# ZooMEISTER/vickers-hardness-Unet

Measured on AMD Instinct MI355X. Metric: 512x512 images/sec (train fwd+bwd), higher is better.
Workload: dtype bf16

## Files before the change

include/vk_unet.h:

```cpp
#ifndef VK_UNET_H
#define VK_UNET_H

#include <stddef.h>
#include <stdint.h>

#ifdef __cplusplus
extern "C" {
#endif

#define VK_ABI_VERSION 1
#define VK_STATS_REPLICAS 32

typedef enum { VK_F32 = 0, VK_BF16 = 1, VK_F16 = 2 } vk_dtype;

enum { VK_OK = 0, VK_ERR_ARG = -1, VK_ERR_STATE = -2, VK_ERR_UNSUPPORTED = -3 };

int vk_version(void);
const char* vk_last_error_string(void);
int vk_has_gfx950_code(void);
int vk_probe_mfma_rate(int iters, int waves_per_simd, float* sink, double* flops_out, void* stream);
int vk_set_reserved_cus(int n);
int vk_debug_hold_cus(int workgroups, int threads, int lds_bytes, int microseconds, const void* traffic, size_t traffic_bytes,
                      float* sink, void* stream);

int vk_debug_set_stamp_buffer(void* device_buffer);
int vk_prof_enable(int on);
int vk_prof_collect(char* buf, size_t buflen);


typedef struct {
  const void* ptr;
  int C;
  int up;
  const float* scale;
  const float* shift;
  int relu;
} vk_src;

typedef struct {
  vk_dtype dtype;
  int N, H, W;
  int Ho, Wo;
  int K;
  int R, S, stride, pad;
  int transposed;
  vk_src src0, src1;
} vk_conv_desc;

int vk_conv_fwd(const vk_conv_desc* d, const void* w, void* y, void* y1, int split_k1, int accumulate,
                double* stats, void* stream);

int vk_conv_dgrad_pool2(const vk_conv_desc* d, const void* w, void* y_half, void* y1, int split_k1, int accumulate,
                        void* stream);

int vk_halo_pack(vk_dtype dtype, int rows, int red, const void* src, void* dst, void* stream);
int vk_conv_uses_halo_pack(const vk_conv_desc* d);
int vk_conv_fwd_packed(const vk_conv_desc* d, const void* w_halo, void* y, void* y1, int split_k1, int accumulate, double* stats,
                       void* stream);

#define VK_SPLITK_WORKSPACE_BYTES (32u << 20)
int vk_conv_fwd_splitk(const vk_conv_desc* d, const void* w_halo, void* y, void* workspace, size_t workspace_bytes, void* stream);

typedef struct {
  const void* z;
  const float* scale;
  const float* shift;
  double* sums;
  const void* mask;
  int accumulate;
} vk_bnr;

int vk_conv_dgrad_fused(const vk_conv_desc* d, const void* w, void* y, void* y1, int split_k1, int pool2, const vk_bnr* bnr,
                        void* stream);

int vk_conv1x1_fwd(const vk_conv_desc* d, const void* w, void* y, int accumulate, double* stats, void* stream);
int vk_conv1x1_wgrad(const vk_conv_desc* d, const void* dz, float* dw, void* workspace, size_t workspace_bytes, void* stream);

int vk_stem_fwd(vk_dtype dtype, int N, int H, int W, const void* x4, const void* wp, void* y, double* stats,
                void* stream);

#define VK_WGRAD_WORKSPACE_BYTES (64u << 20)
int vk_conv_wgrad(const vk_conv_desc* d, const void* dz, float* dw, void* workspace, size_t workspace_bytes, void* stream);
#define VK_WGRAD_BATCH_TABLE_BYTES (128u << 10)
int vk_conv_wgrad_batch_supports(const vk_conv_desc* d);
int vk_conv_wgrad_batch(const vk_conv_desc* descs, const void* const* dz, float* const* dw, int n, int workgroups, void* tables,
                        size_t tables_bytes, void* workspace, size_t workspace_bytes, void* stream);
int vk_stem_wgrad(vk_dtype dtype, int N, int H, int W, const void* x4, const void* dz, float* dw_krsc3, void* workspace,
                  size_t workspace_bytes, void* stream);
int vk_stem_wgrad_bn(vk_dtype dtype, int N, int H, int W, const void* x4, const void* g, const void* z, const float* coef_abc,
                     float* dw_krsc3, void* workspace, size_t workspace_bytes, void* stream);
int vk_stem_dgrad(vk_dtype dtype, int N, int H, int W, const void* g, const void* z, const float* coef_abc, const float* w_krsc3,
                  float* dx, void* stream);

typedef struct {
  int h, w;
  int src_stride;
  int size;
  int nh, nw;
  int top, left;
  int pad_value;
} vk_letterbox_desc;

int vk_letterbox_preprocess(const vk_letterbox_desc* d, const uint8_t* bgr, float* x_nchw, void* stream);
int vk_letterbox_postprocess_mask(const vk_letterbox_desc* d, const float* logits, float thresh, uint8_t* mask_hw, void* stream);
int vk_letterbox_postprocess_prob(const vk_letterbox_desc* d, const float* logits, float* prob_hw, void* stream);
int vk_letterbox_postprocess_labels(const vk_letterbox_desc* d, int C, const float* logits, uint8_t* labels_hw, void* stream);
int vk_letterbox_postprocess_mask_multi(const vk_letterbox_desc* d, int C, const float* logits, float thresh, uint8_t* masks_chw,
                                        void* stream);
int vk_letterbox_postprocess_prob_multi(const vk_letterbox_desc* d, int C, int mode, const float* logits, float* probs_chw, void* stream);

typedef struct {
  int h, w;
  float bin_thresh;
  int morph_kernel;
  int open_iter;
  int close_iter;
  int min_area;
  int max_components;
} vk_geom_desc;

typedef struct {
  int label;
  int area;
  int box[8];
  float cx, cy;
  float rw, rh;
  float ux, uy;
  int hull_n;
  int reserved;
  double d1, d2, d_mean;
} vk_geom_det;

int64_t vk_geom_workspace_bytes(const vk_geom_desc* d, int batch);
int vk_geom_minarearect(const vk_geom_desc* d, int batch, const float* prob, uint8_t* clean, vk_geom_det* dets, int* counts,
                        void* workspace, size_t workspace_bytes, void* stream);

typedef struct {
  int label;
  int area;
  int box[8];
  float cx, cy;
  int valid;
  int branch;
  int n_candidates;
  int contour_n;
  int hull_n;
  int flags;
  double quality;
  double d1, d2, d_mean;
} vk_geom_quad;

int vk_geom_quadrilateral(const vk_geom_desc* d, int fit_outset_px, int batch, const float* prob, uint8_t* clean, vk_geom_quad* dets,
                          int* counts, void* workspace, size_t workspace_bytes, void* stream);

typedef struct {
  int d4;
  int rotate;
  float cos_a, sin_a;
  int photo;
  float alpha, beta;
  int blur_ksize;
  float noise_scale;
  uint32_t noise_seed;
  int clahe_limit;
} vk_aug_params;

#define VK_AUG_TABLE_INTS (256 + 4097 + 4097)
size_t vk_augment_workspace_bytes(int n, int size);

int vk_letterbox_u8(const vk_letterbox_desc* d, const uint8_t* bgr, uint8_t* rgb_sq, void* stream);
int vk_letterbox_mask_u8(const vk_letterbox_desc* d, const uint8_t* mask_hw, uint8_t* mask_sq, void* stream);
int vk_augment_batch(int n, int size, int n_items, const uint8_t* images_rgb, const uint8_t* masks, const int* index_dev,
                     const vk_aug_params* params_host, void* params_dev, const int* color_tables, void* workspace,
// ... 198 lines not shown
```

vickers-hardness-unet_amd/_lib.py:

```python
from __future__ import annotations

import ctypes as C
import os
import subprocess
from pathlib import Path

PKG_DIR = Path(__file__).resolve().parent
LIB_PATH = Path(os.environ["VK_LIB"]) if os.environ.get("VK_LIB") else PKG_DIR / "libvkunet.so"
CSRC = PKG_DIR / "csrc"

VK_F32, VK_BF16, VK_F16 = 0, 1, 2
VK_LOSS_BINARY, VK_LOSS_MULTILABEL, VK_LOSS_MULTICLASS = 0, 1, 2
VK_ENC_RESNET18, VK_ENC_RESNET34, VK_ENC_RESNET50 = 18, 34, 50


class VkError(RuntimeError):
    pass


class vk_src(C.Structure):
    _fields_ = [("ptr", C.c_void_p), ("C", C.c_int), ("up", C.c_int), ("scale", C.c_void_p),
                ("shift", C.c_void_p), ("relu", C.c_int)]


# ... 12 lines not shown
    _fields_ = [("h", C.c_int), ("w", C.c_int), ("src_stride", C.c_int), ("size", C.c_int), ("nh", C.c_int),
                ("nw", C.c_int), ("top", C.c_int), ("left", C.c_int), ("pad_value", C.c_int)]


class vk_geom_desc(C.Structure):
    _fields_ = [("h", C.c_int), ("w", C.c_int), ("bin_thresh", C.c_float), ("morph_kernel", C.c_int), ("open_iter", C.c_int),
                ("close_iter", C.c_int), ("min_area", C.c_int), ("max_components", C.c_int)]


class vk_geom_det(C.Structure):
    _fields_ = [("label", C.c_int), ("area", C.c_int), ("box", C.c_int * 8), ("cx", C.c_float), ("cy", C.c_float),
                ("rw", C.c_float), ("rh", C.c_float), ("ux", C.c_float), ("uy", C.c_float), ("hull_n", C.c_int),
                ("reserved", C.c_int), ("d1", C.c_double), ("d2", C.c_double), ("d_mean", C.c_double)]


class vk_geom_quad(C.Structure):
    _fields_ = [("label", C.c_int), ("area", C.c_int), ("box", C.c_int * 8), ("cx", C.c_float), ("cy", C.c_float),
                ("valid", C.c_int), ("branch", C.c_int), ("n_candidates", C.c_int), ("contour_n", C.c_int), ("hull_n", C.c_int),
                ("flags", C.c_int), ("quality", C.c_double), ("d1", C.c_double), ("d2", C.c_double), ("d_mean", C.c_double)]


class vk_aug_params(C.Structure):
    _fields_ = [("d4", C.c_int), ("rotate", C.c_int), ("cos_a", C.c_float), ("sin_a", C.c_float), ("photo", C.c_int),
                ("alpha", C.c_float), ("beta", C.c_float), ("blur_ksize", C.c_int), ("noise_scale", C.c_float),
                ("noise_seed", C.c_uint32), ("clahe_limit", C.c_int)]


class vk_seg_loss_cfg(C.Structure):
    _fields_ = [("struct_size", C.c_uint32), ("mode", C.c_int32), ("terms", C.c_uint32), ("has_ignore", C.c_int32),
                ("ignore_index", C.c_int32), ("w_pix", C.c_float), ("w_focal", C.c_float), ("w_dice", C.c_float),
                ("w_jaccard", C.c_float), ("w_tversky", C.c_float), ("pix_smooth", C.c_float), ("pix_denom_valid", C.c_int32),
                ("has_pos_weight", C.c_int32), ("pos_weight", C.c_float * 16), ("focal_has_alpha", C.c_int32),
                ("focal_alpha", C.c_float), ("focal_gamma", C.c_float),
                ("dice_smooth", C.c_float), ("dice_eps", C.c_float), ("dice_log", C.c_int32), ("dice_classes", C.c_uint32),
                ("jaccard_smooth", C.c_float), ("jaccard_eps", C.c_float), ("jaccard_log", C.c_int32), ("jaccard_classes", C.c_uint32),
                ("tversky_smooth", C.c_float), ("tversky_eps", C.c_float), ("tversky_log", C.c_int32), ("tversky_classes", C.c_uint32),
                ("tversky_alpha", C.c_float), ("tversky_beta", C.c_float), ("tversky_gamma", C.c_float),
                ("w_mcc", C.c_float), ("mcc_eps", C.c_float)]


class vk_lovasz_cfg(C.Structure):
    _fields_ = [("struct_size", C.c_uint32), ("mode", C.c_int32), ("per_image", C.c_int32), ("has_ignore", C.c_int32),
                ("ignore_index", C.c_int32)]


class vk_unet_config(C.Structure):
    _fields_ = [("N", C.c_int), ("size", C.c_int), ("dtype", C.c_int), ("training", C.c_int), ("width", C.c_int)]


class vk_tensor_info(C.Structure):
    _fields_ = [("name", C.c_char * 96), ("kind", C.c_int), ("dims", C.c_int * 4), ("ndim", C.c_int),
                ("offset", C.c_int64), ("numel", C.c_int64)]


vp, ci, cf, cd, sz, i64 = C.c_void_p, C.c_int, C.c_float, C.c_double, C.c_size_t, C.c_int64
P = C.POINTER

SIGNATURES = {
    "vk_version": (ci, []),
    "vk_last_error_string": (C.c_char_p, []),
    "vk_has_gfx950_code": (ci, []),
    "vk_probe_mfma_rate": (ci, [ci, ci, vp, P(C.c_double), vp]),
    "vk_set_reserved_cus": (ci, [ci]),
    "vk_debug_hold_cus": (ci, [ci, ci, ci, ci, vp, sz, vp, vp]),
    "vk_debug_set_stamp_buffer": (ci, [vp]),
    "vk_prof_enable": (ci, [ci]),
    "vk_prof_collect": (ci, [C.c_char_p, sz]),
    "vk_conv_fwd": (ci, [P(vk_conv_desc), vp, vp, vp, ci, ci, vp, vp]),
    "vk_conv_dgrad_pool2": (ci, [P(vk_conv_desc), vp, vp, vp, ci, ci, vp]),
    "vk_conv_dgrad_fused": (ci, [P(vk_conv_desc), vp, vp, vp, ci, ci, P(vk_bnr), vp]),
    "vk_head_bwd_fused": (ci, [ci, ci, ci, ci, P(vk_src), vp, vp, vp, vp, vp, P(vk_bnr), vp, sz, vp]),
    "vk_halo_pack": (ci, [ci, ci, ci, vp, vp, vp]),
    "vk_conv_uses_halo_pack": (ci, [P(vk_conv_desc)]),
    "vk_conv_fwd_packed": (ci, [P(vk_conv_desc), vp, vp, vp, ci, ci, vp, vp]),
    "vk_conv_fwd_splitk": (ci, [P(vk_conv_desc), vp, vp, vp, sz, vp]),
    "vk_stem_fwd": (ci, [ci, ci, ci, ci, vp, vp, vp, vp, vp]),
    "vk_conv_wgrad": (ci, [P(vk_conv_desc), vp, vp, vp, sz, vp]),
    "vk_conv1x1_fwd": (ci, [P(vk_conv_desc), vp, vp, ci, vp, vp]),
    "vk_conv1x1_wgrad": (ci, [P(vk_conv_desc), vp, vp, vp, sz, vp]),
    "vk_conv_wgrad_batch_supports": (ci, [P(vk_conv_desc)]),
    "vk_conv_wgrad_batch": (ci, [P(vk_conv_desc), P(vp), P(vp), ci, ci, vp, sz, vp, sz, vp]),
    "vk_stem_wgrad": (ci, [ci, ci, ci, ci, vp, vp, vp, vp, sz, vp]),
    "vk_stem_wgrad_bn": (ci, [ci, ci, ci, ci, vp, vp, vp, vp, vp, vp, sz, vp]),
    "vk_stem_dgrad": (ci, [ci, ci, ci, ci, vp, vp, vp, vp, vp, vp]),
    "vk_letterbox_preprocess": (ci, [P(vk_letterbox_desc), vp, vp, vp]),
    "vk_letterbox_postprocess_mask": (ci, [P(vk_letterbox_desc), vp, cf, vp, vp]),
    "vk_letterbox_postprocess_prob": (ci, [P(vk_letterbox_desc), vp, vp, vp]),
    "vk_letterbox_postprocess_labels": (ci, [P(vk_letterbox_desc), ci, vp, vp, vp]),
    "vk_letterbox_postprocess_mask_multi": (ci, [P(vk_letterbox_desc), ci, vp, cf, vp, vp]),
    "vk_letterbox_postprocess_prob_multi": (ci, [P(vk_letterbox_desc), ci, ci, vp, vp, vp]),
    "vk_geom_workspace_bytes": (i64, [P(vk_geom_desc), ci]),
    "vk_geom_minarearect": (ci, [P(vk_geom_desc), ci, vp, vp, vp, vp, vp, sz, vp]),
    "vk_geom_quadrilateral": (ci, [P(vk_geom_desc), ci, ci, vp, vp, vp, vp, vp, sz, vp]),
    "vk_letterbox_u8": (ci, [P(vk_letterbox_desc), vp, vp, vp]),
    "vk_letterbox_mask_u8": (ci, [P(vk_letterbox_desc), vp, vp, vp]),
    "vk_augment_workspace_bytes": (C.c_size_t, [ci, ci]),
    "vk_augment_batch": (ci, [ci, ci, ci, vp, vp, vp, P(vk_aug_params), vp, vp, vp, C.c_size_t, vp, vp, vp]),
    "vk_input_transform": (ci, [ci, ci, ci, ci, vp, vp, vp]),
    "vk_bn_finalize": (ci, [ci, ci, vp, cd, vp, vp, vp, vp, cf, cf, vp, vp, vp, vp, vp]),
    "vk_bn_relu_maxpool": (ci, [ci, ci, ci, ci, ci, vp, vp, vp, vp, vp, vp]),
    "vk_maxpool_bwd": (ci, [ci, ci, ci, ci, ci, vp, vp, vp, vp]),
    "vk_maxpool_bwd_bn_reduce": (ci, [ci, ci, ci, ci, ci, vp, vp, vp, vp, vp, vp, vp, vp]),
    "vk_bn_add_relu": (ci, [ci, sz, ci, vp, vp, vp, vp, vp, vp, vp, vp]),
    "vk_bn_bwd_reduce": (ci, [ci, sz, ci, vp, vp, ci, vp, vp, vp, vp, vp]),
    "vk_bn_bwd_coeffs": (ci, [ci, vp, cd, vp, vp, vp, vp, vp, vp, vp]),
    "vk_bn_bwd_coeffs_frozen": (ci, [ci, vp, vp, vp, vp, vp, vp, vp, vp]),
    "vk_bn_bwd_apply": (ci, [ci, sz, ci, vp, vp, ci, vp, vp, vp, vp, vp, vp, ci, vp]),
    "vk_bn_bwd_apply_fused": (ci, [ci, sz, ci, vp, vp, ci, vp, vp, vp, vp, cd, vp, vp, vp, vp, vp, vp, vp, ci, vp]),
    "vk_upsample2x_bwd": (ci, [ci, ci, ci, ci, ci, vp, vp, ci, vp]),
    "vk_head_fwd": (ci, [ci, ci, ci, ci, P(vk_src), vp, vp, vp, vp]),
    "vk_dec4_tail_eval": (ci, [ci, ci, ci, ci, P(vk_src), vp, vp, vp, vp, vp, vp, vp, vp, vp, vp]),
    "vk_head_bwd": (ci, [ci, ci, ci, ci, P(vk_src), vp, vp, vp, vp, vp, vp, sz, vp]),
    "vk_bce_dice_loss": (ci, [sz, vp, vp, vp, vp, vp, cf, cf, cf, vp]),
    "vk_head_fwd_multi": (ci, [ci, ci, ci, ci, ci, P(vk_src), vp, vp, vp, vp]),
    "vk_head_multi_workspace_bytes": (sz, [ci]),
    "vk_head_bwd_multi": (ci, [ci, ci, ci, ci, ci, P(vk_src), vp, vp, vp, vp, vp, P(vk_bnr), vp, sz, vp]),
    "vk_multi_loss_workspace_bytes": (sz, [ci, ci, ci]),
    "vk_multilabel_loss": (ci, [ci, ci, ci, vp, vp, vp, sz, vp, vp, cf, cf, cf, vp]),
    "vk_multiclass_loss": (ci, [ci, ci, ci, vp, vp, vp, sz, vp, vp, cf, cf, cf, vp]),
    "vk_seg_loss_cfg_size": (sz, []),
    "vk_seg_loss_workspace_bytes": (sz, [ci, ci, ci]),
    "vk_seg_loss": (ci, [P(vk_seg_loss_cfg), ci, ci, ci, vp, vp, vp, sz, vp, vp, cf, vp]),
    "vk_lovasz_cfg_size": (sz, []),
    "vk_lovasz_workspace_bytes": (sz, [P(vk_lovasz_cfg), ci, ci, ci]),
    "vk_lovasz_loss": (ci, [P(vk_lovasz_cfg), ci, ci, ci, vp, vp, vp, sz, vp, vp, cf, ci, vp]),
    "vk_lovasz_flat_workspace_bytes": (sz, [ci, i64]),
    "vk_lovasz_flat": (ci, [vp, vp, ci, i64, vp, sz, vp, vp, vp, vp]),
    "vk_seg_metrics_workspace_bytes": (C.c_size_t, [ci]),
    "vk_seg_metrics": (ci, [ci, sz, vp, vp, ci, cf, cf, vp, sz, vp, vp]),
    "vk_seg_metrics_multi_workspace_bytes": (sz, [ci, ci]),
    "vk_seg_metrics_multi": (ci, [ci, ci, ci, sz, vp, vp, ci, cf, cf, vp, sz, vp, vp, vp, vp]),
    "vk_adamw_step": (ci, [sz, vp, vp, vp, vp, cf, cf, cf, cf, cf, ci, cf, vp, vp, ci, vp]),
    "vk_amp_check_inf": (ci, [sz, vp, vp, vp]),
    "vk_amp_unscale_check": (ci, [sz, vp, vp, vp, vp]),
    "vk_adamw_step_amp": (ci, [sz, vp, vp, vp, vp, cf, cf, cf, cf, cf, vp, cf, vp, vp, vp, vp, ci, vp]),
    "vk_adamw_segment_blocks": (ci, [ci, P(i64), P(C.c_int32), ci]),
    "vk_adamw_step_amp_segments": (ci, [ci, vp, ci, vp, vp, vp, vp, vp, cf, cf, cf, cf, cf, vp, cf, vp, vp, vp, vp]),
    "vk_unet_create": (ci, [P(vk_unet_config), P(vp)]),
    "vk_unet_create_ex": (ci, [P(vk_unet_config), ci, P(vp)]),
    "vk_unet_num_classes": (ci, [vp]),
    "vk_unet_create_enc": (ci, [P(vk_unet_config), ci, ci, P(vp)]),
    "vk_unet_encoder": (ci, [vp]),
    "vk_unet_destroy": (None, [vp]),
    "vk_unet_set_side_stream": (ci, [vp, ci]),
    "vk_unet_num_tensors": (ci, [vp]),
    "vk_unet_tensor_info": (ci, [vp, ci, P(vk_tensor_info)]),
    "vk_unet_param_numel": (i64, [vp]),
    "vk_unet_buffer_numel": (i64, [vp]),
    "vk_unet_workspace_bytes": (i64, [vp]),
    "vk_unet_num_buckets": (ci, [vp]),
    "vk_unet_bucket_range": (ci, [vp, ci, P(i64), P(i64)]),
    "vk_unet_bind": (ci, [vp, vp, vp, vp, vp, vp, sz]),
    "vk_unet_refresh_weights": (ci, [vp, vp]),
    "vk_unet_forward": (ci, [vp, vp, vp, ci, vp]),
    "vk_unet_loss": (ci, [vp, vp, vp, vp, cf, cf, cf, vp]),
    "vk_unet_loss_ex": (ci, [vp, ci, vp, vp, vp, cf, cf, cf, vp]),
    "vk_unet_loss_cfg": (ci, [vp, P(vk_seg_loss_cfg), vp, vp, vp, cf, vp]),
    "vk_unet_loss_lovasz": (ci, [vp, P(vk_seg_loss_cfg), P(vk_lovasz_cfg), cf, vp, vp, vp, sz, vp, cf, vp]),
    "vk_unet_backward": (ci, [vp, vp, ci, ci, vp]),
    "vk_unet_set_trainable": (ci, [vp, P(C.c_uint8), ci]),
    "vk_unet_set_bn_frozen": (ci, [vp, P(C.c_uint8), ci]),
    "vk_unet_set_input_grad": (ci, [vp, vp]),
    "vk_unet_zero_grad": (ci, [vp, vp]),
    "vk_unet_debug_tensor": (ci, [vp, C.c_char_p, P(vp), P(ci * 4)]),
    "vk_comm_unique_id": (ci, [vp]),
    "vk_comm_init": (ci, [ci, ci, vp, P(vp)]),
# ... 78 lines not shown
```

vickers-hardness-unet_amd/csrc/engine.hip:

```cpp
#include <stdarg.h>
#include <stdio.h>
#include <stdlib.h>
#include <string.h>

#include <algorithm>
#include <atomic>
#include <map>
#include <mutex>
#include <string>
#include <vector>

#include "vk_common.h"

namespace vkh {
static thread_local char g_err[512] = "";
void set_error(const char* fmt, ...) {
  va_list ap;
  va_start(ap, fmt);
  vsnprintf(g_err, sizeof(g_err), fmt, ap);
  va_end(ap);
}

struct ProfRec {
  std::string tag;
// ... 1234 lines not shown
                  void* g_out, int g_acc, hipStream_t st) {
  static const int maxc = getenv("VK_BN_APPLY_FUSED_MAXC") ? atoi(getenv("VK_BN_APPLY_FUSED_MAXC")) : VK_BN_APPLY_FUSED_MAXC_DEFAULT;
  if (frozen(h, b)) {
    if (trains(h, b.g_t) || trains(h, b.b_t))
      RET_IF(vk_bn_bwd_coeffs_frozen(C, b.bsums, h->params + b.g_off, b.mean, b.invstd, dgamma_of(h, b), dbeta_of(h, b), b.coef, st));
    return vk_bn_bwd_apply(h->cfg.dtype, pixels, C, dy, z, mask_mode, b.scale, b.shift, mask_src, b.coef, dz, g_out, g_acc, st);
  }
  if (C <= maxc)
    return vk_bn_bwd_apply_fused(h->cfg.dtype, pixels, C, dy, z, mask_mode, b.scale, b.shift, mask_src, b.bsums, b.count, h->params + b.g_off,
                                 b.mean, b.invstd, dgamma_of(h, b), dbeta_of(h, b), dz, g_out, g_acc, st);
  RET_IF(vk_bn_bwd_coeffs(C, b.bsums, b.count, h->params + b.g_off, b.mean, b.invstd, dgamma_of(h, b), dbeta_of(h, b), b.coef, st));
  return vk_bn_bwd_apply(h->cfg.dtype, pixels, C, dy, z, mask_mode, b.scale, b.shift, mask_src, b.coef, dz, g_out, g_acc, st);
}

int bn_relu_bwd_inplace(vk_unet* h, ConvL& c, bool prereduced, hipStream_t st) {
  BnL& b = h->bns[c.bn];
  const size_t pixels = (size_t)h->cfg.N * c.Hout * c.Wout;
  if (!prereduced && bn_sums_needed(h, b)) RET_IF(vk_bn_bwd_reduce(h->cfg.dtype, pixels, c.K, c.g, c.z, 1, b.scale, b.shift, nullptr, b.bsums, st));
  return bn_bwd_phase2(h, b, c.K, pixels, c.g, c.z, prereduced ? 0 : 1, nullptr, c.g, nullptr, 0, st);
}

int wgrad_stream(vk_unet* h, hipStream_t st, hipStream_t* out) {
  *out = st;
  if (!h->side) return VK_OK;
  VK_CHECK_HIP(hipEventRecord(h->ev_fork, st));
  VK_CHECK_HIP(hipStreamWaitEvent(h->side, h->ev_fork, 0));
  h->side_dirty = true;
  *out = h->side;
  return VK_OK;
}

int join_side(vk_unet* h, hipStream_t st) {
  if (!h->side || !h->side_dirty) return VK_OK;
  VK_CHECK_HIP(hipEventRecord(h->ev_join, h->side));
  VK_CHECK_HIP(hipStreamWaitEvent(st, h->ev_join, 0));
  h->side_dirty = false;
  return VK_OK;
}

int conv_wgrad(vk_unet* h, ConvL& c, const vk_src& s0, const vk_src& s1, hipStream_t st) {
  vk_conv_desc d = conv_desc(h, c, s0, s1);
  if (!h->side && vk::wgrad_batch_supports(&d)) {
    h->pending.push_back(vk_unet::WItem{d, c.g, h->grads + c.w_off});
    return VK_OK;
  }
  hipStream_t ws;
  RET_IF(wgrad_stream(h, st, &ws));
  return vk_conv_wgrad(&d, c.g, h->grads + c.w_off, h->ws + h->off_wslab, VK_WGRAD_WORKSPACE_BYTES, ws);
}

vk_bnr bnr_of(vk_unet* h, ConvL& target) {
  BnL& b = h->bns[target.bn];
  vk_bnr r;
  r.z = target.z; r.scale = b.scale; r.shift = b.shift; r.sums = b.bsums; r.mask = nullptr; r.accumulate = 0;
  return r;
}

vk_conv_desc dgrad_desc(vk_unet* h, ConvL& c) {
  vk_conv_desc d;
  d.dtype = h->cfg.dtype;
  d.N = h->cfg.N; d.H = c.Hout; d.W = c.Wout; d.Ho = c.Hin; d.Wo = c.Win;
  d.K = c.Cin; d.R = c.R; d.S = c.R; d.stride = c.stride; d.pad = c.pad; d.transposed = 1;
  vk_src s;
  s.ptr = c.g; s.C = c.K; s.up = 0; s.scale = nullptr; s.shift = nullptr; s.relu = 0;
  d.src0 = s;
  d.src1 = null_src();
  return d;
}

int conv_dgrad_into(vk_unet* h, ConvL& c, ConvL& into, bool* fused, hipStream_t st) {
  vk_conv_desc d = dgrad_desc(h, c);
  if (on_1x1(c)) {
    *fused = false;
    return vk_conv1x1_fwd(&d, dgrad_weights(h, c), into.g, 0, nullptr, st);
  }
  vk_bnr r = bnr_of(h, into);
  int rc = getenv("VK_NO_BNR_FUSION") ? VK_ERR_UNSUPPORTED : vk_conv_dgrad_fused(&d, dgrad_weights(h, c), into.g, nullptr, 0, 0, &r, st);
  *fused = rc == VK_OK;
  if (rc != VK_ERR_UNSUPPORTED) return rc;
  if (c.halo_dg) return vk_conv_fwd_packed(&d, dgrad_weights(h, c), into.g, nullptr, 0, 0, nullptr, st);
  return vk_conv_fwd(&d, dgrad_weights(h, c), into.g, nullptr, 0, 0, nullptr, st);
}

int conv_dgrad(vk_unet* h, ConvL& c, void* y, void* y1, int split, int accumulate, hipStream_t st) {
  vk_conv_desc d;
  d.dtype = h->cfg.dtype;
  d.N = h->cfg.N; d.H = c.Hout; d.W = c.Wout; d.Ho = c.Hin; d.Wo = c.Win;
  d.K = c.Cin; d.R = c.R; d.S = c.R; d.stride = c.stride; d.pad = c.pad; d.transposed = 1;
  vk_src s;
  s.ptr = c.g; s.C = c.K; s.up = 0; s.scale = nullptr; s.shift = nullptr; s.relu = 0;
  d.src0 = s;
  d.src1 = null_src();
  if (on_1x1(c) && !split) return vk_conv1x1_fwd(&d, dgrad_weights(h, c), y, accumulate, nullptr, st);
  if (c.halo_dg) return vk_conv_fwd_packed(&d, dgrad_weights(h, c), y, y1, split, accumulate, nullptr, st);
  return vk_conv_fwd(&d, dgrad_weights(h, c), y, y1, split, accumulate, nullptr, st);
}

int backward_decoder(vk_unet* h, int i, hipStream_t st) {
  DecL& d = h->decs[i];
  ConvL& c1 = h->convs[d.conv1];
  ConvL& c2 = h->convs[d.conv2];
  const int N = h->cfg.N;
  ConvL& stem = h->convs[h->stem_conv];
  Act xprev, skip{nullptr, 0, nullptr, nullptr, 0};
  void* g_prev;
  if (i == 0) {
    BlockL& f5 = h->blocks[h->layer_last_block[3]];
    xprev = Act{f5.out, f5.C, nullptr, nullptr, 0};
    g_prev = f5.gout;
  } else {
    ConvL& pc2 = h->convs[h->decs[i - 1].conv2];
    xprev = bn_act(h, pc2);
    g_prev = pc2.g;
  }
  void* g_skip = nullptr;
  if (i <= 2) {
    BlockL& fb = h->blocks[h->layer_last_block[2 - i]];
    skip = Act{fb.out, fb.C, nullptr, nullptr, 0};
    g_skip = fb.gout;
  } else if (i == 3) {
    skip = bn_act(h, stem);
    g_skip = stem.g;
  }
  const BnL& bn1 = h->bns[c1.bn];
  if (!need_from(h, h->bns[c2.bn].rank)) {
    if (i > 0) h->g_prereduced[h->decs[i - 1].conv2] = 0;
    return VK_OK;
  }
  RET_IF(bn_relu_bwd_inplace(h, c2, h->g_prereduced[d.conv2] != 0, st));
  const bool into1 = need_from(h, bn1.rank);
  bool fused1 = false;
  if (into1) RET_IF(conv_dgrad_into(h, c2, c1, &fused1, st));
  if (trains(h, c2.w_t)) RET_IF(conv_wgrad(h, c2, to_src(bn_act(h, c1)), null_src(), st));
  if (i > 0) h->g_prereduced[h->decs[i - 1].conv2] = 0;
  if (!into1) return VK_OK;
  RET_IF(bn_relu_bwd_inplace(h, c1, fused1, st));
  if (need_from(h, c1.rank + 1)) {
    vk_conv_desc dd = dgrad_desc(h, c1);
    vk_bnr r;
    const bool want_bnr = i > 0 && !getenv("VK_NO_BNR_FUSION");
    if (want_bnr) r = bnr_of(h, h->convs[h->decs[i - 1].conv2]);
    const int rc = vk_conv_dgrad_fused(&dd, dgrad_weights(h, c1), g_prev, d.Cskip ? g_skip : nullptr, d.Cskip ? d.Cup : 0, 1,
                                       want_bnr ? &r : nullptr, st);
    if (rc == VK_OK && want_bnr) h->g_prereduced[h->decs[i - 1].conv2] = 1;
    if (rc != VK_OK && rc != VK_ERR_UNSUPPORTED) return rc;
    if (rc == VK_ERR_UNSUPPORTED) {
      void* dup = h->ws + h->off_dup;
      if (d.Cskip) RET_IF(conv_dgrad(h, c1, dup, g_skip, d.Cup, 0, st));
      else RET_IF(conv_dgrad(h, c1, dup, nullptr, 0, 0, st));
      RET_IF(vk_upsample2x_bwd(h->cfg.dtype, N, d.H, d.W, d.Cup, dup, g_prev, 0, st));
    }
  }
  if (!trains(h, c1.w_t)) return VK_OK;
  return conv_wgrad(h, c1, to_src(xprev, 1), d.Cskip ? to_src(skip) : null_src(), st);
}

int backward_block(vk_unet* h, int bi, hipStream_t st) {
  BlockL& k = h->blocks[bi];
  ConvL& c1 = h->convs[k.conv1];
  ConvL& c2 = h->convs[k.conv2];
  BnL& b2 = h->bns[c2.bn];
  const vk_dtype dt = h->cfg.dtype;
  const size_t pixels = (size_t)h->cfg.N * k.Hout * k.Wout;
  if (!need_from(h, b2.rank)) {
    h->tail_prereduced[(size_t)bi] = 0;
    return VK_OK;
  }
  Act xin;
  void* gin;
  if (bi == 0) {
    xin = Act{h->ws + h->off_pool, 64, nullptr, nullptr, 0};
    gin = h->ws + h->off_gpool;
  } else {
    BlockL& pb = h->blocks[bi - 1];
    xin = Act{pb.out, pb.C, nullptr, nullptr, 0};
    gin = pb.gout;
  }
  const bool pre = h->tail_prereduced[(size_t)bi] != 0;
  h->tail_prereduced[(size_t)bi] = 0;
  if (bi > 0) h->tail_prereduced[(size_t)bi - 1] = 0;
  const int mm = pre ? 0 : 2;
  if (!pre && bn_sums_needed(h, b2)) RET_IF(vk_bn_bwd_reduce(dt, pixels, k.C, k.gout, c2.z, 2, nullptr, nullptr, k.out, b2.bsums, st));
  if (k.convd < 0) {
    RET_IF(bn_bwd_phase2(h, b2, k.C, pixels, k.gout, c2.z, mm, k.out, c2.g, gin, k.in_has_grad_first ? 1 : 0, st));
  } else {
    ConvL& cd = h->convs[k.convd];
    BnL& bd = h->bns[cd.bn];
    RET_IF(bn_bwd_phase2(h, b2, k.C, pixels, k.gout, c2.z, mm, k.out, c2.g, nullptr, 0, st));
    if (bn_sums_needed(h, bd)) RET_IF(vk_bn_bwd_reduce(dt, pixels, k.C, k.gout, cd.z, mm, nullptr, nullptr, k.out, bd.bsums, st));
    RET_IF(bn_bwd_phase2(h, bd, k.C, pixels, k.gout, cd.z, mm, k.out, cd.g, nullptr, 0, st));
  }
  const bool into1 = need_from(h, h->bns[c1.bn].rank);
  bool fused1 = false;
  if (into1) RET_IF(conv_dgrad_into(h, c2, c1, &fused1, st));
  if (trains(h, c2.w_t)) RET_IF(conv_wgrad(h, c2, to_src(bn_act(h, c1)), null_src(), st));
  if (!into1) return k.convd >= 0 && trains(h, h->convs[k.convd].w_t) ? conv_wgrad(h, h->convs[k.convd], to_src(xin), null_src(), st) : VK_OK;
  RET_IF(bn_relu_bwd_inplace(h, c1, fused1, st));
  const bool into_gin = need_from(h, c1.rank + 1);
  bool tail_fused = false;
  const int tail_maxc = getenv("VK_TAIL_BNR_MAXC") ? atoi(getenv("VK_TAIL_BNR_MAXC")) : 1 << 20;
  if (into_gin && k.convd < 0 && bi > 0 && c1.halo_dg && k.C <= tail_maxc && !getenv("VK_NO_TAIL_BNR_FUSION")) {
    BlockL& pb = h->blocks[bi - 1];
    ConvL& pc2 = h->convs[pb.conv2];
    vk_conv_desc dd = dgrad_desc(h, c1);
    vk_bnr r;
    r.z = pc2.z; r.scale = nullptr; r.shift = nullptr; r.sums = h->bns[pc2.bn].bsums; r.mask = pb.out; r.accumulate = 1;
    const int rc = vk_conv_dgrad_fused(&dd, dgrad_weights(h, c1), gin, nullptr, 0, 0, &r, st);
    if (rc == VK_OK) { tail_fused = true; h->tail_prereduced[(size_t)bi - 1] = 1; }
    else if (rc != VK_ERR_UNSUPPORTED) return rc;
  }
  if (into_gin && !tail_fused) RET_IF(conv_dgrad(h, c1, gin, nullptr, 0, 1, st));
  if (k.convd >= 0) {
    ConvL& cd = h->convs[k.convd];
    if (into_gin) RET_IF(conv_dgrad(h, cd, gin, nullptr, 0, 1, st));
    if (trains(h, c1.w_t)) RET_IF(conv_wgrad(h, c1, to_src(xin), null_src(), st));
    return trains(h, cd.w_t) ? conv_wgrad(h, cd, to_src(xin), null_src(), st) : VK_OK;
// ... 197 lines not shown
```

Before: 3011.

## Fuse BN backward, dgrad, wgrad and BN-relu stats into one streaming kernel

Result: faster. 3072 (median of 6 runs) (+2.0%).

```diff
diff --git a/include/vk_unet.h b/include/vk_unet.h
--- a/include/vk_unet.h
+++ b/include/vk_unet.h
@@ -89,6 +89,8 @@
                   size_t workspace_bytes, void* stream);
 int vk_stem_wgrad_bn(vk_dtype dtype, int N, int H, int W, const void* x4, const void* g, const void* z, const float* coef_abc,
                      float* dw_krsc3, void* workspace, size_t workspace_bytes, void* stream);
+int vk_conv_bwd_onepass(const vk_conv_desc* d_fwd, const void* g, const void* z, const float* coef_abc, const void* w_dgrad, void* y,
+                        const vk_bnr* bnr, float* dw, void* workspace, size_t workspace_bytes, void* stream);
 int vk_stem_dgrad(vk_dtype dtype, int N, int H, int W, const void* g, const void* z, const float* coef_abc, const float* w_krsc3,
                   float* dx, void* stream);
 
diff --git a/vickers-hardness-unet_amd/_lib.py b/vickers-hardness-unet_amd/_lib.py
--- a/vickers-hardness-unet_amd/_lib.py
+++ b/vickers-hardness-unet_amd/_lib.py
@@ -118,6 +118,7 @@
     "vk_conv_wgrad_batch": (ci, [P(vk_conv_desc), P(vp), P(vp), ci, ci, vp, sz, vp, sz, vp]),
     "vk_stem_wgrad": (ci, [ci, ci, ci, ci, vp, vp, vp, vp, sz, vp]),
     "vk_stem_wgrad_bn": (ci, [ci, ci, ci, ci, vp, vp, vp, vp, vp, vp, sz, vp]),
+    "vk_conv_bwd_onepass": (ci, [P(vk_conv_desc), vp, vp, vp, vp, vp, P(vk_bnr), vp, vp, sz, vp]),
     "vk_stem_dgrad": (ci, [ci, ci, ci, ci, vp, vp, vp, vp, vp, vp]),
     "vk_letterbox_preprocess": (ci, [P(vk_letterbox_desc), vp, vp, vp]),
     "vk_letterbox_postprocess_mask": (ci, [P(vk_letterbox_desc), vp, cf, vp, vp]),
diff --git a/vickers-hardness-unet_amd/csrc/conv_bwd_onepass.hip b/vickers-hardness-unet_amd/csrc/conv_bwd_onepass.hip
--- /dev/null
+++ b/vickers-hardness-unet_amd/csrc/conv_bwd_onepass.hip
@@ -0,0 +1,402 @@
+#include <stdlib.h>
+
+#include <string>
+#include <type_traits>
+
+#include "vk_common.h"
+
+namespace vk {
+
+void launch_slab_reduce(size_t n4, int splits, const float* slab, float* dw, hipStream_t st);
+
+struct OnePassParams {
+  const void *g, *z, *z1, *w;
+  void* y;
+  const float *coef, *scale, *shift, *bnr_scale, *bnr_shift;
+  double* sums;
+  float* slab;
+  int N, H, W, RS, RSsum, relu;
+  uint32_t w_bytes, t_bytes;
+};
+
+template <int CK>
+struct OnePassCfg {
+  static constexpr int NSTEP = CK == 16 ? 5 : 9;
+  static constexpr int APS = CK == 16 ? 48 : 96;
+  static constexpr int VPP = CK / 8;
+  static constexpr int NVEC = 18 * VPP;
+  static constexpr int NLD = (NVEC + 63) / 64;
+  static constexpr int ROWB = CK == 16 ? 1024 : 2048;
+  static constexpr int V_OFF = 4 * ROWB, ZERO_OFF = 8 * ROWB;
+  static constexpr int WAVE_LDS = 8 * ROWB + 64;
+  static constexpr int RED = CK * 9 * CK * 4;
+  static constexpr int SMEM = 4 * WAVE_LDS > RED ? 4 * WAVE_LDS : RED;
+  static_assert(18 * APS <= ROWB && NLD <= 2, "row image");
+};
+
+template <typename T, int CK>
+__global__ __launch_bounds__(256, (CK == 16 ? 2 : 1)) void conv_bwd_onepass_kernel(const OnePassParams p) {
+  using Cfg = OnePassCfg<CK>;
+  constexpr int NSTEP = Cfg::NSTEP, APS = Cfg::APS, VPP = Cfg::VPP, NVEC = Cfg::NVEC, NLD = Cfg::NLD, ROWB = Cfg::ROWB;
+  constexpr int VE = 8, TC = CK / 16;
+  static_assert(sizeof(T) == 2, "16-bit element types");
+  extern __shared__ __attribute__((aligned(16))) char smem[];
+  typedef __attribute__((address_space(3))) s16x4_t* lds_s16x4_ptr;
+  const int RS = p.RS;
+  const int tid = threadIdx.x, lane = tid & 63;
+  const int wave = __builtin_amdgcn_readfirstlane(tid >> 6);
+  char* const ring = smem + wave * Cfg::WAVE_LDS;
+  char* const vring = ring + Cfg::V_OFF;
+  const int strips_x = (p.W + 15) / 16, strips_y = (p.H + RS - 1) / RS;
+  int sid = (int)blockIdx.x * 4 + wave;
+  const bool active = sid < p.N * strips_y * strips_x;
+  const int strip = sid;
+  const int sx = sid % strips_x;
+  sid /= strips_x;
+  const int sy = sid % strips_y;
+  const int n = sid / strips_y;
+  const int x0 = sx * 16, ys = sy * RS, ye = min(p.H, ys + RS);
+  const int li = lane & 15, kg = lane >> 4;
+
+  f32x4_t wacc[9][TC][TC];
+#pragma unroll
+  for (int t = 0; t < 9; ++t)
+#pragma unroll
+    for (int a = 0; a < TC; ++a)
+#pragma unroll
+      for (int b = 0; b < TC; ++b) wacc[t][a][b] = f32x4_t{0.f, 0.f, 0.f, 0.f};
+
+  if (active) {
+    const __amdgpu_buffer_rsrc_t rsg = make_rsrc(p.g, p.t_bytes);
+    const __amdgpu_buffer_rsrc_t rsz = make_rsrc(p.z, p.t_bytes);
+    const __amdgpu_buffer_rsrc_t rs1 = make_rsrc(p.z1, p.t_bytes);
+    const __amdgpu_buffer_rsrc_t rsw = make_rsrc(p.w, p.w_bytes);
+
+    u32x4_t wf[NSTEP][TC];
+#pragma unroll
+    for (int st = 0; st < NSTEP; ++st)
+#pragma unroll
+      for (int a = 0; a < TC; ++a) {
+        const int row = a * 16 + li;
+        uint32_t off;
+        bool ok = true;
+        if (CK == 16) {
+          const int tap = 2 * st + (kg >> 1);
+          ok = tap < 9;
+          off = (uint32_t)(((row * 9 + (8 - tap)) * 16 + (kg & 1) * VE) * 2);
+        } else {
+          const int pos = kg ^ (((row >> 2) & 1) << 1);
+          off = (uint32_t)((((8 - st) * CK + row) * 4 + pos) * 16);
+        }
+        wf[st][a] = buf_load16(rsw, ok ? off : kOOB);
+      }
+    if (lane < 4) *reinterpret_cast<u32x4_t*>(ring + Cfg::ZERO_OFF + lane * 16) = u32x4_t{0, 0, 0, 0};
+
+    int st_off[NLD], ld_col[NLD];
+    bool xok[NLD];
+#pragma unroll
+    for (int q = 0; q < NLD; ++q) {
+      const int v = lane + 64 * q;
+      int hx = v / VPP, hv = v % VPP;
+      if (VPP == 4) {
+        if ((hx | 3) < 18) hx = (hx & ~3) | ((hx & 1) << 1) | ((hx >> 1) & 1);
+      } else {
+        if ((v | 15) < NVEC) { hx = (v & 7) | ((v >> 4) << 3); hv = (v >> 3) & 1; }
+      }
+      const int xs = x0 - 1 + hx;
+      xok[q] = v < NVEC && (unsigned)xs < (unsigned)p.W;
+      ld_col[q] = xs * CK + hv * VE;
+      st_off[q] = v < NVEC ? hx * APS + hv * 16 : -1;
+    }
+    static_assert(VPP == 4 || NLD == 1, "C = 16: one staged vector per lane");
+    const int hvl = VPP == 4 ? lane % VPP : (((lane | 15) < NVEC) ? (lane >> 3) & 1 : lane % VPP);
+    const bool aff = p.scale != nullptr, relu = p.relu != 0;
+    float sc[VE], sh[VE], ca[VE], cb[VE], cc[VE];
+#pragma unroll
+    for (int j = 0; j < VE; ++j) {
+      sc[j] = aff ? p.scale[hvl * VE + j] : 1.f;
+      sh[j] = aff ? p.shift[hvl * VE + j] : 0.f;
+      ca[j] = p.coef[hvl * VE + j];
+      cb[j] = p.coef[CK + hvl * VE + j];
+      cc[j] = p.coef[2 * CK + hvl * VE + j];
+    }
+    struct RowQ {
+      u32x4_t g[NLD], z[NLD], v[NLD];
+    };
+    auto issue = [&](int j, RowQ& r) {
+      const bool rok = (unsigned)j < (unsigned)p.H;
+#pragma unroll
+      for (int q = 0; q < NLD; ++q) {
+        const uint32_t off = (rok && xok[q]) ? (uint32_t)(((n * p.H + j) * p.W) * CK + ld_col[q]) * 2u : kOOB;
+        r.g[q] = buf_load16(rsg, off);
+        r.z[q] = buf_load16(rsz, off);
+        r.v[q] = buf_load16(rs1, off);
+      }
+    };
+    auto write_row = [&](int j, const RowQ& r) {
+      const bool rok = (unsigned)j < (unsigned)p.H;
+      const int slot = (j & 3) * ROWB;
+#pragma unroll
+      for (int q = 0; q < NLD; ++q) {
+        if (st_off[q] < 0) continue;
+        float gf[VE], zf[VE], o[VE];
+        Vec16<T>::unpack(r.g[q], gf);
+        Vec16<T>::unpack(r.z[q], zf);
+#pragma unroll
+        for (int e = 0; e < VE; ++e) o[e] = fmaf(ca[e], gf[e], fmaf(cb[e], zf[e], cc[e]));
+        u32x4_t dz = Vec16<T>::pack(o);
+        u32x4_t v = r.v[q];
+        if (aff) v = AffineRelu<T>::run(v, sc, sh, relu);
+        if (!(rok && xok[q])) {
+          dz = u32x4_t{0, 0, 0, 0};
+          v = u32x4_t{0, 0, 0, 0};
+        }
+        *reinterpret_cast<u32x4_t*>(ring + slot + st_off[q]) = dz;
+        *reinterpret_cast<u32x4_t*>(vring + slot + st_off[q]) = v;
+      }
+    };
+
+    int fr_r16[CK == 16 ? NSTEP : 1], fr_off16[CK == 16 ? NSTEP : 1];
+    if (CK == 16) {
+#pragma unroll
+      for (int st = 0; st < NSTEP; ++st) {
+        const int tap = 2 * st + (kg >> 1);
+        const int r = tap / 3, sxx = tap - r * 3;
+        fr_r16[st] = tap < 9 ? r : -100;
+        fr_off16[st] = (li + sxx) * APS + (kg & 1) * 16;
+      }
+    }
+    const int fr_base32 = kg * 16;
+    const int lane_t = (4 * kg + (li >> 2)) * APS + (4 * (lane & 3)) * 2;
+    auto tr = [](const char* q) { return __builtin_bit_cast(u32x2_t, __builtin_amdgcn_ds_read_tr16_b64_v4i16((lds_s16x4_ptr)(q))); };
+
+    const int xo = x0 + li;
+    const bool x_ok = xo < p.W;
+    float bsc[TC][4], bsh[TC][4], s1[TC][4], s2[TC][4];
+#pragma unroll
+    for (int a = 0; a < TC; ++a)
+#pragma unroll
+      for (int e = 0; e < 4; ++e) {
+        const int ch = a * 16 + kg * 4 + e;
+        bsc[a][e] = p.bnr_scale[ch];
+        bsh[a][e] = p.bnr_shift[ch];
+        s1[a][e] = 0.f; s2[a][e] = 0.f;
+      }
+    auto round_t = [&](float (&f)[4]) {
+      float g[8] = {f[0], f[1], f[2], f[3], 0.f, 0.f, 0.f, 0.f};
+      const u32x4_t pk = Vec16<T>::pack(g);
+      Vec16<T>::unpack(pk, g);
+#pragma unroll
+      for (int e = 0; e < 4; ++e) f[e] = g[e];
+      return u32x2_t{pk[0], pk[1]};
+    };
+    const uint32_t lane_ob = x_ok ? (uint32_t)(((n * p.H) * p.W + xo) * CK + kg * 4) * 2u : kOOB;
+    const uint32_t row_ob = (uint32_t)(p.W * CK * 2);
+    auto out_off = [&](int a, int y) -> uint32_t { return lane_ob + (uint32_t)y * row_ob + (uint32_t)(a * 32); };
+    u32x2_t zq[2][TC];
+    auto z_issue = [&](int y, u32x2_t (&z)[TC]) {
+      const bool ok = y < p.H;
+#pragma unroll
+      for (int a = 0; a < TC; ++a) z[a] = __builtin_amdgcn_raw_buffer_load_b64(rs1, ok ? out_off(a, y) : kOOB, 0, 0);
+    };
+    auto finish = [&](int a, float (&f)[4], uint32_t boff, bool counted, u32x2_t zr) {
+      float zf[8];
+      Vec16<T>::unpack(u32x4_t{zr[0], zr[1], 0u, 0u}, zf);
+#pragma unroll
+      for (int e = 0; e < 4; ++e) {
+        if (!counted || !(fmaf(zf[e], bsc[a][e], bsh[a][e]) > 0.f)) f[e] = 0.f;
+        s1[a][e] += f[e];
+        s2[a][e] += f[e] * zf[e];
+      }
+      const u32x2_t pk = round_t(f);
+      if ((int32_t)boff >= 0) *reinterpret_cast<u32x2_t*>((char*)p.y + boff) = pk;
+    };
+
+    RowQ pre[4];
+    issue(ys - 1, pre[3]);
+    issue(ys, pre[0]);
+    issue(ys + 1, pre[1]);
+    issue(ys + 2, pre[2]);
+    z_issue(ys, zq[0]);
+    write_row(ys - 1, pre[3]);
+    issue(ys + 3, pre[3]);
+    write_row(ys, pre[0]);
+    auto row = [&](int y, auto ph_c) {
+      constexpr int PH = decltype(ph_c)::value;
+      write_row(y + 1, pre[(PH + 1) & 3]);
+      issue(y + 4, pre[PH & 3]);
+      z_issue(y + 1, zq[(PH & 1) ^ 1]);
+      f32x4_t acc[TC];
+#pragma unroll
+      for (int a = 0; a < TC; ++a) acc[a] = f32x4_t{0.f, 0.f, 0.f, 0.f};
+#pragma unroll
+      for (int st = 0; st < NSTEP; ++st) {
+        int addr;
+        if (CK == 16) {
+          const int vrow = y - 1 + fr_r16[st];
+          addr = fr_r16[st] < 0 ? Cfg::ZERO_OFF : (vrow & 3) * ROWB + fr_off16[st];
+        } else {
+          const int r = st / 3, sxx = st - r * 3;
+          addr = ((y - 1 + r) & 3) * ROWB + (li + sxx) * APS + fr_base32;
+        }
+        const u32x4_t xf = *reinterpret_cast<const u32x4_t*>(ring + addr);
+#pragma unroll
+        for (int a = 0; a < TC; ++a) acc[a] = Mma<T>::run(wf[st][a], xf, acc[a]);
+      }
+      __builtin_amdgcn_sched_barrier(0);
+      const bool y_ok = y < p.H;
+#pragma unroll
+      for (int a = 0; a < TC; ++a) {
+        float f[4] = {acc[a][0], acc[a][1], acc[a][2], acc[a][3]};
+        (void)round_t(f);
+        finish(a, f, y_ok ? out_off(a, y) : kOOB, x_ok && y_ok, zq[PH & 1][a]);
+      }
+      if constexpr ((PH & 1) == 1) {
+        constexpr int SL = (PH + 3) & 3, SH = PH & 3;
+        u32x4_t zf[TC];
+#pragma unroll
+        for (int a = 0; a < TC; ++a) {
+          const u32x2_t lo = tr(ring + SL * ROWB + APS + lane_t + a * 32), hi = tr(ring + SH * ROWB + APS + lane_t + a * 32);
+          zf[a] = u32x4_t{lo[0], lo[1], hi[0], hi[1]};
+        }
+#pragma unroll
+        for (int r = 0; r < 3; ++r) {
+          const int slo = ((PH + 2 + r) & 3) * ROWB, shi = ((PH + 3 + r) & 3) * ROWB;
+#pragma unroll
+          for (int s_ = 0; s_ < 3; ++s_) {
+            u32x4_t vf[TC];
+#pragma unroll
+            for (int b = 0; b < TC; ++b) {
+              const u32x2_t lo = tr(vring + slo + s_ * APS + lane_t + b * 32), hi = tr(vring + shi + s_ * APS + lane_t + b * 32);
+              vf[b] = u32x4_t{lo[0], lo[1], hi[0], hi[1]};
+            }
+#pragma unroll
+            for (int a = 0; a < TC; ++a)
+#pragma unroll
+              for (int b = 0; b < TC; ++b) wacc[r * 3 + s_][a][b] = Mma<T>::run(zf[a], vf[b], wacc[r * 3 + s_][a][b]);
+          }
+        }
+      }
+    };
+    double* const sp = p.sums + (size_t)(strip % VK_STATS_REPLICAS) * 2 * CK;
+    auto flush_sums = [&]() {
+#pragma unroll
+      for (int a = 0; a < TC; ++a)
+#pragma unroll
+        for (int e = 0; e < 4; ++e) {
+          const float u = row16_sum(s1[a][e]), v = row16_sum(s2[a][e]);
+          const int ch = a * 16 + kg * 4 + e;
+          if (li == 0) {
+            atomicAdd(sp + ch, (double)u);
+            atomicAdd(sp + CK + ch, (double)v);
+          }
+          s1[a][e] = 0.f; s2[a][e] = 0.f;
+        }
+    };
+    const int RSsum = p.RSsum;
+    for (int yb = ys, left = RSsum; yb < ye; yb += 4) {
+      row(yb, std::integral_constant<int, 0>{});
+      row(yb + 1, std::integral_constant<int, 1>{});
+      row(yb + 2, std::integral_constant<int, 2>{});
+      row(yb + 3, std::integral_constant<int, 3>{});
+      left -= 4;
+      if (left == 0 || yb + 4 >= ye) {
+        flush_sums();
+        left = RSsum;
+      }
+    }
+  }
+
+  __syncthreads();
+  float* const red = reinterpret_cast<float*>(smem);
+#pragma unroll 1
+  for (int phase = 0; phase < 4; ++phase) {
+    if (wave == phase) {
+#pragma unroll
+      for (int t = 0; t < 9; ++t)
+#pragma unroll
+        for (int a = 0; a < TC; ++a)
+#pragma unroll
+          for (int b = 0; b < TC; ++b)
+#pragma unroll
+            for (int e = 0; e < 4; ++e) {
+              const int k = a * 16 + kg * 4 + e, c = b * 16 + li;
+              float* dst = red + (k * 9 + t) * CK + c;
+              if (phase > 0) *dst += wacc[t][a][b][e];
+              else *dst = wacc[t][a][b][e];
+            }
+    }
+    __syncthreads();
+  }
+  float* const slab = p.slab + (size_t)blockIdx.x * CK * 9 * CK;
+  for (int i = tid; i < CK * 9 * CK / 4; i += 256) *reinterpret_cast<f32x4_t*>(slab + i * 4) = *reinterpret_cast<const f32x4_t*>(red + i * 4);
+}
+
+template <typename T, int CK>
+static int launch_onepass(OnePassParams p, float* dw, size_t slab_bytes, hipStream_t st) {
+  using Cfg = OnePassCfg<CK>;
+  const char* e_rs = getenv("VK_STREAM_RS");
+  int RS = 256;
+  if (e_rs) {
+    RS = atoi(e_rs);
+  } else {
+    const long per_row_block = (long)p.N * ((p.W + 15) / 16), resident = CK == 16 ? 2048 : 1024;
+    while (RS > 32 && per_row_block * ((p.H + RS - 1) / RS) < resident) RS >>= 1;
+  }
+  RS = (RS + 7) & ~7;
+  if (RS < 8) RS = 8;
+  int RSsum = RS;
+  if (!e_rs) {
+    const long per_row_block = (long)p.N * ((p.W + 15) / 16);
+    RSsum = 32;
+    while (RSsum * 2 <= 256 && per_row_block * ((p.H + 2 * RSsum - 1) / (2 * RSsum)) >= 4096) RSsum *= 2;
+    if (RS < RSsum) RS = RSsum;
+  }
+  p.RSsum = RSsum;
+  p.RS = RS;
+  const long strips = (long)p.N * ((p.H + RS - 1) / RS) * ((p.W + 15) / 16);
+  const long nwg = (strips + 3) / 4;
+  if ((size_t)nwg * CK * 9 * CK * sizeof(float) > slab_bytes) return VK_ERR_UNSUPPORTED;
+  static bool attr_done = false;
+  if (!attr_done && Cfg::SMEM > 64 * 1024) {
+    VK_CHECK_HIP(hipFuncSetAttribute((const void*)conv_bwd_onepass_kernel<T, CK>, hipFuncAttributeMaxDynamicSharedMemorySize, Cfg::SMEM));
+    attr_done = true;
+  }
+  {
+    static const std::string tag = std::string("bwd_onepass_16b_c") + std::to_string(CK);
+    const double px = (double)p.N * p.H * p.W;
+    vkh::ProfScope ps(tag.c_str(), st, 2.0 * 2.0 * px * CK * 9.0 * CK, 4.0 * px * CK * 2.0 + 9.0 * CK * CK * (2.0 + 4.0));
+    hipLaunchKernelGGL((conv_bwd_onepass_kernel<T, CK>), dim3((unsigned)nwg), dim3(256), Cfg::SMEM, st, p);
+  }
+  launch_slab_reduce((size_t)CK * 9 * CK / 4, (int)nwg, p.slab, dw, st);
+  VK_CHECK_HIP(hipGetLastError());
+  return VK_OK;
+}
+
+}
+
+extern "C" int vk_conv_bwd_onepass(const vk_conv_desc* d, const void* g, const void* z, const float* coef_abc, const void* w_dgrad, void* y,
+                                   const vk_bnr* bnr, float* dw, void* workspace, size_t workspace_bytes, void* stream) {
+  VK_CHECK_ARG(d && g && z && coef_abc && w_dgrad && y && bnr && dw, "vk_conv_bwd_onepass: null argument");
+  if (d->dtype != VK_BF16 && d->dtype != VK_F16) return VK_ERR_UNSUPPORTED;
+  if (d->R != 3 || d->S != 3 || d->stride != 1 || d->pad != 1 || d->transposed || d->H != d->Ho || d->W != d->Wo) return VK_ERR_UNSUPPORTED;
+  if (d->src1.ptr || d->src0.up || d->src0.C != d->K || (d->K != 16 && d->K != 32)) return VK_ERR_UNSUPPORTED;
+  if ((size_t)d->N * d->H * d->W * d->K * 2 >= (1ull << 31)) return VK_ERR_UNSUPPORTED;
+  if (!workspace || (reinterpret_cast<uintptr_t>(workspace) & 15)) return VK_ERR_UNSUPPORTED;
+  VK_CHECK_ARG(d->src0.ptr && d->N > 0 && d->H > 0 && d->W > 0, "vk_conv_bwd_onepass: empty descriptor");
+  VK_CHECK_ARG((d->src0.scale != nullptr) == (d->src0.shift != nullptr), "vk_conv_bwd_onepass: scale and shift come together");
+  VK_CHECK_ARG(bnr->z == d->src0.ptr && !bnr->mask && !bnr->accumulate && bnr->sums && bnr->scale && bnr->shift,
+               "vk_conv_bwd_onepass: bnr must describe the layer's own input (z = src0.ptr, scale, shift, sums; no mask, no accumulate)");
+  vk::OnePassParams p;
+  p.g = g; p.z = z; p.z1 = d->src0.ptr; p.w = w_dgrad; p.y = y;
+  p.coef = coef_abc; p.scale = d->src0.scale; p.shift = d->src0.shift; p.relu = d->src0.relu;
+  p.bnr_scale = bnr->scale; p.bnr_shift = bnr->shift; p.sums = bnr->sums;
+  p.slab = (float*)workspace;
+  p.N = d->N; p.H = d->H; p.W = d->W; p.RS = 0;
+  p.w_bytes = (uint32_t)((size_t)d->K * 9 * d->K * 2);
+  p.t_bytes = (uint32_t)((size_t)d->N * d->H * d->W * d->K * 2);
+  hipStream_t st = (hipStream_t)stream;
+  if (d->dtype == VK_BF16)
+    return d->K == 16 ? vk::launch_onepass<vk::bf16_t, 16>(p, dw, workspace_bytes, st) : vk::launch_onepass<vk::bf16_t, 32>(p, dw, workspace_bytes, st);
+  return d->K == 16 ? vk::launch_onepass<vk::f16_t, 16>(p, dw, workspace_bytes, st) : vk::launch_onepass<vk::f16_t, 32>(p, dw, workspace_bytes, st);
+}
diff --git a/vickers-hardness-unet_amd/csrc/engine.hip b/vickers-hardness-unet_amd/csrc/engine.hip
--- a/vickers-hardness-unet_amd/csrc/engine.hip
+++ b/vickers-hardness-unet_amd/csrc/engine.hip
@@ -1340,6 +1340,30 @@
   return vk_conv_fwd(&d, dgrad_weights(h, c), into.g, nullptr, 0, 0, nullptr, st);
 }
 
+int conv_bwd_onepass(vk_unet* h, ConvL& c, ConvL& into, int* state, hipStream_t st) {
+  *state = 0;
+  BnL& b = h->bns[c.bn];
+  vk_conv_desc d = conv_desc(h, c, to_src(bn_act(h, into)), null_src());
+  if (d.dtype == VK_F32 || d.R != 3 || d.S != 3 || d.stride != 1 || d.pad != 1 || d.src0.up || d.src0.C != d.K || (d.K != 16 && d.K != 32)) return VK_OK;
+  static const int maxc = getenv("VK_BN_APPLY_FUSED_MAXC") ? atoi(getenv("VK_BN_APPLY_FUSED_MAXC")) : VK_BN_APPLY_FUSED_MAXC_DEFAULT;
+  if (!frozen(h, b) && c.K <= maxc) return VK_OK;
+  if (frozen(h, b)) {
+    if (trains(h, b.g_t) || trains(h, b.b_t))
+      RET_IF(vk_bn_bwd_coeffs_frozen(c.K, b.bsums, h->params + b.g_off, b.mean, b.invstd, dgamma_of(h, b), dbeta_of(h, b), b.coef, st));
+  } else {
+    RET_IF(vk_bn_bwd_coeffs(c.K, b.bsums, b.count, h->params + b.g_off, b.mean, b.invstd, dgamma_of(h, b), dbeta_of(h, b), b.coef, st));
+  }
+  vk_bnr r = bnr_of(h, into);
+  const int rc = vk_conv_bwd_onepass(&d, c.g, c.z, b.coef, dgrad_weights(h, c), into.g, &r, h->grads + c.w_off, h->ws + h->off_wslab,
+                                     VK_WGRAD_WORKSPACE_BYTES, st);
+  if (rc == VK_ERR_UNSUPPORTED) {
+    *state = 2;
+    return vk_bn_bwd_apply(h->cfg.dtype, (size_t)h->cfg.N * c.Hout * c.Wout, c.K, c.g, c.z, 0, b.scale, b.shift, nullptr, b.coef, c.g, nullptr, 0, st);
+  }
+  *state = rc == VK_OK ? 1 : 0;
+  return rc;
+}
+
 int conv_dgrad(vk_unet* h, ConvL& c, void* y, void* y1, int split, int accumulate, hipStream_t st) {
   vk_conv_desc d;
   d.dtype = h->cfg.dtype;
@@ -1385,11 +1409,19 @@
     if (i > 0) h->g_prereduced[h->decs[i - 1].conv2] = 0;
     return VK_OK;
   }
-  RET_IF(bn_relu_bwd_inplace(h, c2, h->g_prereduced[d.conv2] != 0, st));
   const bool into1 = need_from(h, bn1.rank);
   bool fused1 = false;
-  if (into1) RET_IF(conv_dgrad_into(h, c2, c1, &fused1, st));
-  if (trains(h, c2.w_t)) RET_IF(conv_wgrad(h, c2, to_src(bn_act(h, c1)), null_src(), st));
+  int onepass = 0;
+  if (h->g_prereduced[d.conv2] && into1 && trains(h, c2.w_t) && h->cfg.dtype != VK_F32 && !h->side && !on_1x1(c2) && !getenv("VK_NO_ONEPASS") &&
+      !getenv("VK_NO_BNR_FUSION"))
+    RET_IF(conv_bwd_onepass(h, c2, c1, &onepass, st));
+  if (onepass == 1) {
+    fused1 = true;
+  } else {
+    if (onepass == 0) RET_IF(bn_relu_bwd_inplace(h, c2, h->g_prereduced[d.conv2] != 0, st));
+    if (into1) RET_IF(conv_dgrad_into(h, c2, c1, &fused1, st));
+    if (trains(h, c2.w_t)) RET_IF(conv_wgrad(h, c2, to_src(bn_act(h, c1)), null_src(), st));
+  }
   if (i > 0) h->g_prereduced[h->decs[i - 1].conv2] = 0;
   if (!into1) return VK_OK;
   RET_IF(bn_relu_bwd_inplace(h, c1, fused1, st));
```
